# pdeljanov/Symphonia

Measured on AMD Instinct MI355X. Metric: decoded audio frames/sec (batch IMDCT+OLA), higher is better.
Workload: dtype f32

## Files before the change

### symphonia_amd/csrc/aac.hip

```cpp
#include <type_traits>

#include "imdct_wave.h"

namespace symaccel {

namespace {

#ifndef SYM_AAC_VARIANT
#define SYM_AAC_VARIANT 0
#endif
#if SYM_AAC_VARIANT == 1
constexpr int kWaves = 6;
#define SYM_AAC_WAVES_PER_SIMD 3
#else
constexpr int kWaves = 4;
#endif
constexpr int kTabTw = 0;
constexpr int kTabKbd = 1024;
constexpr int kTabSine = 2048;
constexpr int kTabKbdShort = 3072;
constexpr int kTabSineShort = 3200;
constexpr int kTabFloats = 3328;

enum : int { ONLY_LONG = 0, LONG_START = 1, EIGHT_SHORT = 2, LONG_STOP = 3 };
constexpr int kP0 = 512 - 64;
constexpr int kP1 = 512 + 64;

__device__ __forceinline__ void pcm_short4(const float *H, int q0, const float *short_win, const float *prev_short_win,
                                           float (&acc)[4]) {
    const int w = q0 >> 7, i0 = q0 & 127;
    bool have = false;
    if (w >= 1) {
        float a[4];
        ys4(H, w - 1, 128 + i0, a);
        const float4 wr = *reinterpret_cast<const float4 *>(short_win + 124 - i0);
        a[0] *= wr.w; a[1] *= wr.z; a[2] *= wr.y; a[3] *= wr.x;
#pragma unroll
        for (int q = 0; q < 4; ++q) acc[q] = (w - 1 == 0) ? a[q] : (0.0f + a[q]);
        have = true;
    }
    if (w <= 7) {
        float bq[4];
        ys4(H, w, i0, bq);
        const float4 wf = *reinterpret_cast<const float4 *>((w == 0 ? prev_short_win : short_win) + i0);
        bq[0] *= wf.x; bq[1] *= wf.y; bq[2] *= wf.z; bq[3] *= wf.w;
#pragma unroll
        for (int q = 0; q < 4; ++q) acc[q] = have ? (acc[q] + bq[q]) : bq[q];
    }
}

__device__ __forceinline__ void stop_window4(const float *psw, int j0, float *w) {
    float4 v = make_float4(1.0f, 1.0f, 1.0f, 1.0f);
    if (j0 >= kP0 && j0 < kP1) v = *reinterpret_cast<const float4 *>(psw + j0 - kP0);
    w[0] = v.x; w[1] = v.y; w[2] = v.z; w[3] = v.w;
}
__device__ __forceinline__ void start_window4(const float *sw, int j0, float *w) {
    float4 v = make_float4(1.0f, 1.0f, 1.0f, 1.0f);
    if (j0 >= kP0 && j0 < kP1) {
        const float4 r = *reinterpret_cast<const float4 *>(sw + 124 - (j0 - kP0));
        v = make_float4(r.w, r.z, r.y, r.x);
    }
    w[0] = v.x; w[1] = v.y; w[2] = v.z; w[3] = v.w;
}

#if defined(SYM_AAC_WAVES_PER_SIMD) && !defined(SYM_AAC_MIN_WAVES)
#define SYM_AAC_MIN_WAVES SYM_AAC_WAVES_PER_SIMD
#endif
#ifndef SYM_AAC_MIN_WAVES
#define SYM_AAC_MIN_WAVES 2
#endif
#ifndef SYM_AAC_PREFETCH
#define SYM_AAC_PREFETCH 1
#endif
#ifndef SYM_AAC_QUAD
#define SYM_AAC_QUAD 1
#endif
__device__ __forceinline__ float2 ld_line(const float2 *p) { return ld_stream(p); }
__device__ __forceinline__ void st_slot(float *frame, int m2, const float (&v)[8]) {
    float4 *o4 = reinterpret_cast<float4 *>(frame);
    st_stream(o4 + m2, make_float4(v[0], v[1], v[2], v[3]));
    st_stream(o4 + 255 - m2, make_float4(v[4], v[5], v[6], v[7]));
}


#if !SYM_AAC_QUAD
#include "experiments/aac_wave_walk.h"
#endif



constexpr int kSlotOff = kShortRowsEnd;
static_assert(kSlotOff + 1024 <= kWaveLds, "delay slot must fit the per-wave LDS behind the short-window rows");

struct AacJsArgs {
    const int2 *chain;
    const int32_t *pair_chains;
    const symaccel_aac_js_frame *desc;
    AacBandMaps maps;
    unsigned n_chains;
};

template <bool JS>
__global__ __launch_bounds__(256, SYM_AAC_MIN_WAVES) void aac_synth_quad_kernel(
    DevTables tb, const float *__restrict__ coeffs, const uint8_t *__restrict__ side,
    const float *__restrict__ delay_in, float *__restrict__ delay_out, float *__restrict__ pcm,
    unsigned frames_per_chain, unsigned seg_steps, unsigned segs_per_chain, AacJsArgs js) {
    __shared__ __attribute__((aligned(16))) float tabs[kTabFloats];
    __shared__ __attribute__((aligned(16))) float wave_lds[4][kWaveLds];
    constexpr int CH = JS ? 2 : 1;
    __shared__ __attribute__((aligned(16))) float carry[CH][2][1024];
    if constexpr (!JS) {
        if (js.chain && js.chain[blockIdx.x / segs_per_chain].x >= 0) return;
    }
    for (int i = (int)threadIdx.x; i < 1024; i += 256) {
        tabs[kTabTw + i] = reinterpret_cast<const float *>(tb.aac_tw_long)[i];
        tabs[kTabKbd + i] = tb.aac_kbd_long[i];
        tabs[kTabSine + i] = tb.aac_sine_long[i];
        if (i < 128) {
            tabs[kTabKbdShort + i] = tb.aac_kbd_short[i];
            tabs[kTabSineShort + i] = tb.aac_sine_short[i];
        }
    }
    const int lane = (int)threadIdx.x & 63, wave = (int)threadIdx.x >> 6;
    float *ldsf = wave_lds[wave];
    c32 *lds = reinterpret_cast<c32 *>(ldsf);
    const c32 *tw = reinterpret_cast<const c32 *>(tabs + kTabTw);
    const unsigned unit = blockIdx.x / segs_per_chain, seg = blockIdx.x % segs_per_chain;
    const unsigned chain = JS ? (unsigned)js.pair_chains[2 * unit] : unit, chain1 = JS ? (unsigned)js.pair_chains[2 * unit + 1] : unit;
    if constexpr (JS) {
        if (chain >= js.n_chains || chain1 >= js.n_chains || chain == chain1) return;
    }
    const long t_begin = (long)seg * seg_steps * 4;
    const long t_end = t_begin + (long)seg_steps * 4 < (long)frames_per_chain ? t_begin + (long)seg_steps * 4 : (long)frames_per_chain;
    const long n_steps = (t_end - t_begin + 3) / 4;
    const size_t chain_base0 = (size_t)chain * frames_per_chain, chain_base1 = (size_t)chain1 * frames_per_chain;
    LaneTables lt;
    load_lane_tables(tb, lane, lt);

    if (t_begin == 0 && wave == 3) {
#pragma unroll
        for (int ch = 0; ch < CH; ++ch) {
            const float4 *src = reinterpret_cast<const float4 *>(delay_in + (size_t)(ch ? chain1 : chain) * 1024);
#pragma unroll
            for (int q = 0; q < 4; ++q) reinterpret_cast<float4 *>(carry[ch][1])[lane + 64 * q] = src[lane + 64 * q];
        }
    }
    long t_loaded = (wave == 3 && t_begin > 0) ? t_begin - 1 : t_begin + wave;
    float2 line[8];
    unsigned sb_next = 0;
    float2 line1[8];
    uint32_t dq[3] = {0u, 0u, 0u};
    unsigned sb1_next = 0;
    uint32_t sfb_long[2] = {0u, 0u};
    unsigned sfb_short = 0;
    auto fetch1 = [&](long tf, int ln) {
        if constexpr (JS) {
            const float2 *ps = reinterpret_cast<const float2 *>(coeffs + (chain_base1 + (size_t)tf) * 1024);
            const uint32_t *d = reinterpret_cast<const uint32_t *>(js.desc + (size_t)unit * frames_per_chain + (size_t)tf);
#pragma unroll
            for (int s = 0; s < 8; ++s) line1[s] = ld_line(ps + ln + 64 * s);
            dq[0] = d[ln];
            dq[1] = d[ln + 64];
            dq[2] = ln < 33 ? d[ln + 128] : 0u;
            sb1_next = side[chain_base1 + (size_t)tf];
        }
    };
    if constexpr (JS) {
#pragma unroll
        for (int s = 0; s < 8; ++s) sfb_long[s >> 2] |= (uint32_t)js.maps.long4[(lane >> 1) + 32 * s] << (8 * (s & 3));
        sfb_short = js.maps.short4[(lane >> 1) & 31];
    }
    if (t_loaded < t_end) {
        const float2 *src = reinterpret_cast<const float2 *>(coeffs + (chain_base0 + (size_t)t_loaded) * 1024);
#pragma unroll
        for (int s = 0; s < 8; ++s) line[s] = ld_line(src + lane + 64 * s);
        sb_next = side[chain_base0 + (size_t)t_loaded];
        fetch1(t_loaded, lane);
    } else {
        t_loaded = -100;
#pragma unroll
        for (int s = 0; s < 8; ++s) line[s] = make_float2(0.0f, 0.0f);
        if constexpr (JS) {
#pragma unroll
            for (int s = 0; s < 8; ++s) line1[s] = make_float2(0.0f, 0.0f);
        }
    }
    __syncthreads();

    long t = t_begin - 4 + wave;
    const int lane_of_wave = lane;
    for (long i = -1; i < n_steps; ++i, t += 4) {
        int lane = lane_of_wave;
        if constexpr (JS) {
#if defined(__HIP_DEVICE_COMPILE__)
            asm volatile("" : "+v"(lane));
#endif
        }
        const bool active = t == t_loaded;
        const bool emit = i >= 0;
        const unsigned sb0 = sb_next, sb1 = sb1_next;
        if constexpr (JS) {
            if (active) {
                uint32_t *dl = reinterpret_cast<uint32_t *>(ldsf);
                dl[lane] = dq[0];
                dl[lane + 64] = dq[1];
                if (lane < 33) dl[lane + 128] = dq[2];
                wave_sync();
                const unsigned hdr = dl[0];
                const bool one = (hdr & 255u) == 1u;
                const int max_sfb = (int)((hdr >> 8) & 255u);
                const uint8_t *mode = reinterpret_cast<const uint8_t *>(dl + 1);
                const float *scale = reinterpret_cast<const float *>(dl + 33);
#pragma unroll
                for (int s = 0; s < 8; ++s) {
                    const float2 l = line[s], r = line1[s];
                    const int sfb = one ? (int)((sfb_long[s >> 2] >> (8 * (s & 3))) & 255u) : (int)sfb_short;
                    const int slot = one ? sfb : 16 * s + sfb;
                    const bool coded = sfb < max_sfb && slot < 128;
                    const int sl = slot < 127 ? slot : 127;
                    const unsigned m = mode[sl];
                    const float sc = scale[sl];
                    const bool ms = coded && m == SYMACCEL_AAC_JS_MS, is = coded && m == SYMACCEL_AAC_JS_INTENSITY;
                    line[s] = ms ? make_float2(l.x + r.x, l.y + r.y) : l;
                    line1[s] = ms ? make_float2(l.x - r.x, l.y - r.y) : (is ? make_float2(sc * l.x, sc * l.y) : r);
                }
                wave_sync();
            }
        }
        const long tn = t < t_begin ? t_begin + 3 : t + 4;
#pragma unroll 1
        for (int ch = 0; ch < CH; ++ch) {
        if constexpr (JS) {
#if defined(__HIP_DEVICE_COMPILE__)
            asm volatile("" : "+v"(lane));
#endif
        }
        const unsigned sb = ch ? sb1 : sb0;
        const size_t chain_base = ch ? chain_base1 : chain_base0;
        const int seq = (int)(sb & 3u);
        const int shape = (int)((sb >> 2) & 1u), prev_shape = (int)((sb >> 3) & 1u);
        float *my_slot = wave == 3 ? carry[ch][i & 1] : ldsf + kSlotOff;
        const float *prev_slot = wave == 0 ? carry[ch][(i + 1) & 1] : wave_lds[wave - 1] + kSlotOff;
        float xw[2][8];
        auto ln_at = [&](int s) -> float2 {
            if constexpr (JS) return ch ? line1[s] : line[s];
            else return line[s];
        };

        if (active) {
            c32 z[8];
            if (seq != EIGHT_SHORT) {
                const int mirror = (63 - lane) * 4;
#pragma unroll
                for (int s = 0; s < 8; ++s) {
                    const float mirrored = __int_as_float(__builtin_amdgcn_ds_bpermute(mirror, __float_as_int(ln_at(7 - s).y)));
                    z[s] = pre_twiddle(ln_at(s).x, mirrored, tw[lane + 64 * s]);
                }
            } else {
#pragma unroll
                for (int s = 0; s < 8; ++s) {
                    ldsf[short_row(s) + 2 * lane] = ln_at(s).x;
                    ldsf[short_row(s) + 2 * lane + 1] = ln_at(s).y;
                }
                wave_sync();
            }
            if (tn < t_end) {
                if (ch == 0) {
                    sb_next = side[chain_base0 + (size_t)tn];
                    const float2 *src = reinterpret_cast<const float2 *>(coeffs + (chain_base0 + (size_t)tn) * 1024);
#pragma unroll
                    for (int s = 0; s < 8; ++s) line[s] = ld_line(src + lane + 64 * s);
                }
                if (ch == CH - 1) fetch1(tn, lane);
            }
            if (seq != EIGHT_SHORT) {
                fft512_wave(z, lane, lds, lt);
                const float *wprev = tabs + (prev_shape ? kTabKbd : kTabSine);
                const float *wcur = tabs + (shape ? kTabKbd : kTabSine);
#pragma unroll
                for (int h = 0; h < 2; ++h) {
                    const int m2 = lane + 64 * h;
                    float x[8], x2[8];
                    post_slot(lds, tw, m2, x, x2);
                    float wo[8];
                    if (seq == LONG_STOP) {
                        const float *psw = tabs + (prev_shape ? kTabKbdShort : kTabSineShort);
                        stop_window4(psw, 4 * m2, wo);
                        stop_window4(psw, 1020 - 4 * m2, wo + 4);
                    } else {
                        load_slot(wprev, m2, wo);
                    }
#pragma unroll
                    for (int q = 0; q < 8; ++q) xw[h][q] = x[q] * wo[q];
                    float wd[8], nd[8];
                    if (seq == LONG_START) {
                        const float *sw = tabs + (shape ? kTabKbdShort : kTabSineShort);
                        start_window4(sw, 4 * m2, wd);
                        start_window4(sw, 1020 - 4 * m2, wd + 4);
                    } else {
                        float wr[8];
                        load_slot(wcur, m2, wr);
#pragma unroll
                        for (int q = 0; q < 8; ++q) wd[q] = wr[7 - q];
                    }
#pragma unroll
                    for (int q = 0; q < 8; ++q) {
                        const int j = q < 4 ? 4 * m2 + q : 1020 - 4 * m2 + (q - 4);
                        const float v = x2[q] * wd[q];
                        nd[q] = (seq == LONG_START && j >= kP1) ? 0.0f : v;
                    }
                    store_slot(my_slot, m2, nd);
                }
            } else {
                imdct_short_wave(lane, ldsf, tb.aac_tw_short, lt);
                const float *sw = tabs + (shape ? kTabKbdShort : kTabSineShort);
                const float *psw = tabs + (prev_shape ? kTabKbdShort : kTabSineShort);
#pragma unroll 1
                for (int e = 0; e < 4; ++e) {
                    const int j0 = 4 * lane + 256 * e;
                    float nd[4] = {0.0f, 0.0f, 0.0f, 0.0f};
                    if (j0 < kP1) pcm_short4(ldsf, j0 + kP1, sw, psw, nd);
                    *reinterpret_cast<float4 *>(my_slot + j0) = make_float4(nd[0], nd[1], nd[2], nd[3]);
                }
            }
        }
        wg_sync_lds();

        if (active && emit) {
            float *frame_out = pcm + (chain_base + (size_t)t) * 1024;
            if (seq != EIGHT_SHORT) {
#pragma unroll
                for (int h = 0; h < 2; ++h) {
                    const int m2 = lane + 64 * h;
                    float dl[8], dst[8];
                    load_slot(prev_slot, m2, dl);
#pragma unroll
                    for (int q = 0; q < 8; ++q) {
                        const int j = q < 4 ? 4 * m2 + q : 1020 - 4 * m2 + (q - 4);
                        const float v = dl[q] + xw[h][q];
                        dst[q] = (seq == LONG_STOP && j < kP0) ? dl[q] : v;
                    }
                    st_slot(frame_out, m2, dst);
                }
            } else {
                const float *sw = tabs + (shape ? kTabKbdShort : kTabSineShort);
                const float *psw = tabs + (prev_shape ? kTabKbdShort : kTabSineShort);
#pragma unroll 1
                for (int e = 0; e < 4; ++e) {
                    const int j0 = 4 * lane + 256 * e;
                    const float4 d = *reinterpret_cast<const float4 *>(prev_slot + j0);
                    float o[4] = {d.x, d.y, d.z, d.w};
                    if (j0 >= kP0) {
                        float ps[4];
                        pcm_short4(ldsf, j0 - kP0, sw, psw, ps);
#pragma unroll
                        for (int q = 0; q < 4; ++q) o[q] = o[q] + ps[q];
                    }
                    st_stream(reinterpret_cast<float4 *>(frame_out + j0), make_float4(o[0], o[1], o[2], o[3]));
                }
            }
            if (t + 1 == (long)frames_per_chain) {
                float4 *d = reinterpret_cast<float4 *>(delay_out + (size_t)(ch ? chain1 : chain) * 1024);
#pragma unroll
                for (int q = 0; q < 4; ++q) d[lane + 64 * q] = reinterpret_cast<const float4 *>(my_slot)[lane + 64 * q];
            }
        }
        wg_sync_lds();
        }
        if (active) t_loaded = tn < t_end ? tn : -100;
    }
}

__global__ void aac_js_index_kernel(const int32_t *__restrict__ pair_chains, unsigned n_pairs, unsigned n_chains, int2 *__restrict__ chain_index) {
    const unsigned i = blockIdx.x * blockDim.x + threadIdx.x;
    if (i < 2 * n_pairs && (unsigned)pair_chains[i] < n_chains && (unsigned)pair_chains[i ^ 1u] < n_chains)
        chain_index[pair_chains[i]] = make_int2(pair_chains[i ^ 1u], (int)i);
}

}

int launch_aac(symaccel_ctx *ctx, const float *d_coeffs, const uint8_t *d_side, const float *d_delay_in,
               float *d_delay_out, float *d_pcm, size_t n_chains, size_t frames_per_chain, const AacBandMaps *maps,
               const int32_t *d_pair_chains, const symaccel_aac_js_frame *d_js_desc, size_t n_pairs, void *d_js_scratch) {
    if (frames_per_chain > 0x7fffffffu) return SYMACCEL_ERR_INVALID_ARG;
#if SYM_AAC_QUAD
    {
        const size_t steps_per_chain = (frames_per_chain + 3) / 4;
        unsigned seg_steps;
        if (ctx->segment > 0) seg_steps = (unsigned)((ctx->segment + 3) / 4);
        else seg_steps = choose_segment(ctx, n_chains, steps_per_chain, SYM_AAC_MIN_WAVES, 1, 1, 1);
        if (seg_steps > steps_per_chain) seg_steps = (unsigned)steps_per_chain;
        const size_t segs = (steps_per_chain + seg_steps - 1) / seg_steps;
        const size_t grid = n_chains * segs;
        if (grid > 0x7fffffffu) return SYMACCEL_ERR_INVALID_ARG;
        AacJsArgs js{nullptr, nullptr, nullptr, AacBandMaps{}, (unsigned)n_chains};
        if (n_pairs == 0 || !maps) {
            hipLaunchKernelGGL(aac_synth_quad_kernel<false>, dim3((unsigned)grid), dim3(256), 0, ctx->stream, ctx->dev, d_coeffs, d_side,
                               d_delay_in, d_delay_out, d_pcm, (unsigned)frames_per_chain, seg_steps, (unsigned)segs, js);
        } else {
            if (n_pairs * frames_per_chain > 0x7fffffffu) return SYMACCEL_ERR_INVALID_ARG;
            const bool unpaired = 2 * n_pairs < n_chains;
            int2 *chain_index = unpaired ? reinterpret_cast<int2 *>(d_js_scratch) : nullptr;
            if (unpaired) {
                SYM_GPU(ctx, hipMemsetAsync(chain_index, 0xff, n_chains * sizeof(int2), ctx->stream));
                hipLaunchKernelGGL(aac_js_index_kernel, dim3((unsigned)((2 * n_pairs + 255) / 256)), dim3(256), 0, ctx->stream, d_pair_chains,
                                   (unsigned)n_pairs, (unsigned)n_chains, chain_index);
                SYM_GPU(ctx, hipGetLastError());
            }
            js = AacJsArgs{chain_index, d_pair_chains, d_js_desc, *maps, (unsigned)n_chains};
            unsigned pseg_steps;
            if (ctx->segment > 0) pseg_steps = (unsigned)((ctx->segment + 3) / 4);
            else pseg_steps = choose_segment(ctx, n_pairs, steps_per_chain, SYM_AAC_MIN_WAVES, 1, 1, 1);
            if (pseg_steps > steps_per_chain) pseg_steps = (unsigned)steps_per_chain;
            const size_t psegs = (steps_per_chain + pseg_steps - 1) / pseg_steps;
            if (n_pairs * psegs > 0x7fffffffu) return SYMACCEL_ERR_INVALID_ARG;
            hipLaunchKernelGGL(aac_synth_quad_kernel<true>, dim3((unsigned)(n_pairs * psegs)), dim3(256), 0, ctx->stream, ctx->dev, d_coeffs, d_side,
                               d_delay_in, d_delay_out, d_pcm, (unsigned)frames_per_chain, pseg_steps, (unsigned)psegs, js);
            SYM_GPU(ctx, hipGetLastError());
            if (unpaired)
                hipLaunchKernelGGL(aac_synth_quad_kernel<false>, dim3((unsigned)grid), dim3(256), 0, ctx->stream, ctx->dev, d_coeffs, d_side,
                                   d_delay_in, d_delay_out, d_pcm, (unsigned)frames_per_chain, seg_steps, (unsigned)segs, js);
        }
        SYM_GPU(ctx, hipGetLastError());
        return SYMACCEL_OK;
    }
#else
    return launch_aac_wave_walk(ctx, d_coeffs, d_side, d_delay_in, d_delay_out, d_pcm, n_chains, frames_per_chain);
#endif
}

}
```

Baseline: 305.4 million.

## Split quad synth loop into halo, full and ragged steps with specialized tails

Restructures the per-wave step loop into a templated step lambda called as a halo step, a loop of full steps, and a ragged tail. The per-step active, emit and bound checks disappear, and the halo step needs only a wave sync instead of a workgroup barrier. The long-window tail is specialized per window sequence, reusing the previous window when the shapes match. The short-window output is staged through LDS so all paths share one store. It adds readfirstlane scalarization, a scheduling barrier that forces the prefetch to settle, and an optional probe header, at the cost of code size and register pressure.

```diff
diff --git a/symphonia_amd/csrc/aac.hip b/symphonia_amd/csrc/aac.hip
--- a/symphonia_amd/csrc/aac.hip
+++ b/symphonia_amd/csrc/aac.hip
@@ -92,6 +92,17 @@
 constexpr int kSlotOff = kShortRowsEnd;
 static_assert(kSlotOff + 1024 <= kWaveLds, "delay slot must fit the per-wave LDS behind the short-window rows");
 
+enum : int { kStepHalo = 0, kStepFull = 1, kStepRagged = 2 };
+template <int V> using step_kind = std::integral_constant<int, V>;
+
+__device__ __forceinline__ void settle_prefetch(const float2 (&line)[8]) {
+#if defined(__HIP_DEVICE_COMPILE__)
+    __builtin_amdgcn_sched_barrier(0);
+    asm volatile("" : : "v"(line[0].x), "v"(line[0].y), "v"(line[1].x), "v"(line[1].y), "v"(line[2].x), "v"(line[2].y), "v"(line[3].x), "v"(line[3].y),
+                        "v"(line[4].x), "v"(line[4].y), "v"(line[5].x), "v"(line[5].y), "v"(line[6].x), "v"(line[6].y), "v"(line[7].x), "v"(line[7].y));
+#endif
+}
+
 struct AacJsArgs {
     const int2 *chain;
     const int32_t *pair_chains;
@@ -99,6 +110,10 @@
     AacBandMaps maps;
     unsigned n_chains;
 };
+
+#if SYM_AAC_QUAD == 2
+#include "experiments/aac_quad_probe.h"
+#endif
 
 template <bool JS>
 __global__ __launch_bounds__(256, SYM_AAC_MIN_WAVES) void aac_synth_quad_kernel(
@@ -121,7 +136,7 @@
             tabs[kTabSineShort + i] = tb.aac_sine_short[i];
         }
     }
-    const int lane = (int)threadIdx.x & 63, wave = (int)threadIdx.x >> 6;
+    const int lane = (int)threadIdx.x & 63, wave = __builtin_amdgcn_readfirstlane((int)threadIdx.x >> 6);
     float *ldsf = wave_lds[wave];
     c32 *lds = reinterpret_cast<c32 *>(ldsf);
     const c32 *tw = reinterpret_cast<const c32 *>(tabs + kTabTw);
@@ -132,12 +147,13 @@
     }
     const long t_begin = (long)seg * seg_steps * 4;
     const long t_end = t_begin + (long)seg_steps * 4 < (long)frames_per_chain ? t_begin + (long)seg_steps * 4 : (long)frames_per_chain;
-    const long n_steps = (t_end - t_begin + 3) / 4;
+    if (t_end <= t_begin) return;
     const size_t chain_base0 = (size_t)chain * frames_per_chain, chain_base1 = (size_t)chain1 * frames_per_chain;
     LaneTables lt;
     load_lane_tables(tb, lane, lt);
 
-    if (t_begin == 0 && wave == 3) {
+    const bool has_halo = t_begin > 0;
+    if (!has_halo && wave == 3) {
 #pragma unroll
         for (int ch = 0; ch < CH; ++ch) {
             const float4 *src = reinterpret_cast<const float4 *>(delay_in + (size_t)(ch ? chain1 : chain) * 1024);
@@ -145,7 +161,7 @@
             for (int q = 0; q < 4; ++q) reinterpret_cast<float4 *>(carry[ch][1])[lane + 64 * q] = src[lane + 64 * q];
         }
     }
-    long t_loaded = (wave == 3 && t_begin > 0) ? t_begin - 1 : t_begin + wave;
+    const long t_first = (wave == 3 && has_halo) ? t_begin - 1 : t_begin + wave;
     float2 line[8];
     unsigned sb_next = 0;
     float2 line1[8];
@@ -170,14 +186,13 @@
         for (int s = 0; s < 8; ++s) sfb_long[s >> 2] |= (uint32_t)js.maps.long4[(lane >> 1) + 32 * s] << (8 * (s & 3));
         sfb_short = js.maps.short4[(lane >> 1) & 31];
     }
-    if (t_loaded < t_end) {
-        const float2 *src = reinterpret_cast<const float2 *>(coeffs + (chain_base0 + (size_t)t_loaded) * 1024);
+    if (t_first < t_end) {
+        const float2 *src = reinterpret_cast<const float2 *>(coeffs + (chain_base0 + (size_t)t_first) * 1024);
 #pragma unroll
         for (int s = 0; s < 8; ++s) line[s] = ld_line(src + lane + 64 * s);
-        sb_next = side[chain_base0 + (size_t)t_loaded];
-        fetch1(t_loaded, lane);
+        sb_next = side[chain_base0 + (size_t)t_first];
+        fetch1(t_first, lane);
     } else {
-        t_loaded = -100;
 #pragma unroll
         for (int s = 0; s < 8; ++s) line[s] = make_float2(0.0f, 0.0f);
         if constexpr (JS) {
@@ -187,18 +202,17 @@
     }
     __syncthreads();
 
-    long t = t_begin - 4 + wave;
     const int lane_of_wave = lane;
-    for (long i = -1; i < n_steps; ++i, t += 4) {
+    auto step = [&](auto kind_c, int i, long t, bool active) __attribute__((always_inline)) {
+        constexpr int KIND = decltype(kind_c)::value;
         int lane = lane_of_wave;
         if constexpr (JS) {
 #if defined(__HIP_DEVICE_COMPILE__)
             asm volatile("" : "+v"(lane));
 #endif
         }
-        const bool active = t == t_loaded;
-        const bool emit = i >= 0;
-        const unsigned sb0 = sb_next, sb1 = sb1_next;
+        const unsigned sb0 = (unsigned)__builtin_amdgcn_readfirstlane((int)sb_next);
+        const unsigned sb1 = JS ? (unsigned)__builtin_amdgcn_readfirstlane((int)sb1_next) : 0u;
         if constexpr (JS) {
             if (active) {
                 uint32_t *dl = reinterpret_cast<uint32_t *>(ldsf);
@@ -227,7 +241,8 @@
                 wave_sync();
             }
         }
-        const long tn = t < t_begin ? t_begin + 3 : t + 4;
+        const long tn = KIND == kStepHalo ? t_begin + 3 : (t + 4 < t_end ? t + 4 : t);
+        const bool fetch = KIND == kStepFull || (KIND == kStepHalo && tn < t_end);
 #pragma unroll 1
         for (int ch = 0; ch < CH; ++ch) {
         if constexpr (JS) {
@@ -240,12 +255,56 @@
         const int seq = (int)(sb & 3u);
         const int shape = (int)((sb >> 2) & 1u), prev_shape = (int)((sb >> 3) & 1u);
         float *my_slot = wave == 3 ? carry[ch][i & 1] : ldsf + kSlotOff;
-        const float *prev_slot = wave == 0 ? carry[ch][(i + 1) & 1] : wave_lds[wave - 1] + kSlotOff;
+        float *prev_slot = wave == 0 ? carry[ch][(i + 1) & 1] : wave_lds[wave > 0 ? wave - 1 : 0] + kSlotOff;
         float xw[2][8];
         auto ln_at = [&](int s) -> float2 {
             if constexpr (JS) return ch ? line1[s] : line[s];
             else return line[s];
         };
+        auto long_tail = [&](auto seq_c) __attribute__((always_inline)) {
+            constexpr int SEQ = decltype(seq_c)::value;
+            const float *wprev = tabs + (prev_shape ? kTabKbd : kTabSine);
+            const float *wcur = tabs + (shape ? kTabKbd : kTabSine);
+#pragma unroll
+            for (int h = 0; h < 2; ++h) {
+                const int m2 = lane + 64 * h;
+                float x[8], x2[8];
+                post_slot(lds, tw, m2, x, x2);
+                float wo[8];
+                if constexpr (SEQ == LONG_STOP) {
+                    const float *psw = tabs + (prev_shape ? kTabKbdShort : kTabSineShort);
+                    stop_window4(psw, 4 * m2, wo);
+                    stop_window4(psw, 1020 - 4 * m2, wo + 4);
+                } else {
+                    load_slot(wprev, m2, wo);
+                }
+#pragma unroll
+                for (int q = 0; q < 8; ++q) xw[h][q] = x[q] * wo[q];
+                float wd[8], nd[8];
+                if constexpr (SEQ == LONG_START) {
+                    const float *sw = tabs + (shape ? kTabKbdShort : kTabSineShort);
+                    start_window4(sw, 4 * m2, wd);
+                    start_window4(sw, 1020 - 4 * m2, wd + 4);
+                } else {
+                    float wr[8];
+                    if (SEQ == ONLY_LONG && shape == prev_shape) {
+#pragma unroll
+                        for (int q = 0; q < 8; ++q) wr[q] = wo[q];
+                    } else {
+                        load_slot(wcur, m2, wr);
+                    }
+#pragma unroll
+                    for (int q = 0; q < 8; ++q) wd[q] = wr[7 - q];
+                }
+#pragma unroll
+                for (int q = 0; q < 8; ++q) {
+                    const int j = q < 4 ? 4 * m2 + q : 1020 - 4 * m2 + (q - 4);
+                    const float v = x2[q] * wd[q];
+                    nd[q] = (SEQ == LONG_START && j >= kP1) ? 0.0f : v;
+                }
+                store_slot(my_slot, m2, nd);
+            }
+        };
 
         if (active) {
             c32 z[8];
@@ -264,7 +323,7 @@
                 }
                 wave_sync();
             }
-            if (tn < t_end) {
+            if (fetch) {
                 if (ch == 0) {
                     sb_next = side[chain_base0 + (size_t)tn];
                     const float2 *src = reinterpret_cast<const float2 *>(coeffs + (chain_base0 + (size_t)tn) * 1024);
@@ -275,42 +334,9 @@
             }
             if (seq != EIGHT_SHORT) {
                 fft512_wave(z, lane, lds, lt);
-                const float *wprev = tabs + (prev_shape ? kTabKbd : kTabSine);
-                const float *wcur = tabs + (shape ? kTabKbd : kTabSine);
-#pragma unroll
-                for (int h = 0; h < 2; ++h) {
-                    const int m2 = lane + 64 * h;
-                    float x[8], x2[8];
-                    post_slot(lds, tw, m2, x, x2);
-                    float wo[8];
-                    if (seq == LONG_STOP) {
-                        const float *psw = tabs + (prev_shape ? kTabKbdShort : kTabSineShort);
-                        stop_window4(psw, 4 * m2, wo);
-                        stop_window4(psw, 1020 - 4 * m2, wo + 4);
-                    } else {
-                        load_slot(wprev, m2, wo);
-                    }
-#pragma unroll
-                    for (int q = 0; q < 8; ++q) xw[h][q] = x[q] * wo[q];
-                    float wd[8], nd[8];
-                    if (seq == LONG_START) {
-                        const float *sw = tabs + (shape ? kTabKbdShort : kTabSineShort);
-                        start_window4(sw, 4 * m2, wd);
-                        start_window4(sw, 1020 - 4 * m2, wd + 4);
-                    } else {
-                        float wr[8];
-                        load_slot(wcur, m2, wr);
-#pragma unroll
-                        for (int q = 0; q < 8; ++q) wd[q] = wr[7 - q];
-                    }
-#pragma unroll
-                    for (int q = 0; q < 8; ++q) {
-                        const int j = q < 4 ? 4 * m2 + q : 1020 - 4 * m2 + (q - 4);
-                        const float v = x2[q] * wd[q];
-                        nd[q] = (seq == LONG_START && j >= kP1) ? 0.0f : v;
-                    }
-                    store_slot(my_slot, m2, nd);
-                }
+                if (seq == ONLY_LONG) long_tail(step_kind<ONLY_LONG>{});
+                else if (seq == LONG_START) long_tail(step_kind<LONG_START>{});
+                else long_tail(step_kind<LONG_STOP>{});
             } else {
                 imdct_short_wave(lane, ldsf, tb.aac_tw_short, lt);
                 const float *sw = tabs + (shape ? kTabKbdShort : kTabSineShort);
@@ -324,23 +350,29 @@
                 }
             }
         }
+        if constexpr (KIND == kStepHalo) {
+            wave_sync();
+        } else {
         wg_sync_lds();
 
-        if (active && emit) {
+        if (active) {
             float *frame_out = pcm + (chain_base + (size_t)t) * 1024;
+            float dst[2][8];
             if (seq != EIGHT_SHORT) {
 #pragma unroll
                 for (int h = 0; h < 2; ++h) {
                     const int m2 = lane + 64 * h;
-                    float dl[8], dst[8];
+                    float dl[8];
                     load_slot(prev_slot, m2, dl);
 #pragma unroll
-                    for (int q = 0; q < 8; ++q) {
-                        const int j = q < 4 ? 4 * m2 + q : 1020 - 4 * m2 + (q - 4);
-                        const float v = dl[q] + xw[h][q];
-                        dst[q] = (seq == LONG_STOP && j < kP0) ? dl[q] : v;
+                    for (int q = 0; q < 8; ++q) dst[h][q] = dl[q] + xw[h][q];
+                    if (seq == LONG_STOP) {
+#pragma unroll
+                        for (int q = 0; q < 8; ++q) {
+                            const int j = q < 4 ? 4 * m2 + q : 1020 - 4 * m2 + (q - 4);
+                            dst[h][q] = j < kP0 ? dl[q] : dst[h][q];
+                        }
                     }
-                    st_slot(frame_out, m2, dst);
                 }
             } else {
                 const float *sw = tabs + (shape ? kTabKbdShort : kTabSineShort);
@@ -356,9 +388,15 @@
 #pragma unroll
                         for (int q = 0; q < 4; ++q) o[q] = o[q] + ps[q];
                     }
-                    st_stream(reinterpret_cast<float4 *>(frame_out + j0), make_float4(o[0], o[1], o[2], o[3]));
-                }
-            }
+                    *reinterpret_cast<float4 *>(prev_slot + j0) = make_float4(o[0], o[1], o[2], o[3]);
+                }
+                wave_sync();
+#pragma unroll
+                for (int h = 0; h < 2; ++h) load_slot(prev_slot, lane + 64 * h, dst[h]);
+            }
+#pragma unroll
+            for (int h = 0; h < 2; ++h) st_slot(frame_out, lane + 64 * h, dst[h]);
+            if constexpr (KIND == kStepFull && !JS) settle_prefetch(line);
             if (t + 1 == (long)frames_per_chain) {
                 float4 *d = reinterpret_cast<float4 *>(delay_out + (size_t)(ch ? chain1 : chain) * 1024);
 #pragma unroll
@@ -367,8 +405,16 @@
         }
         wg_sync_lds();
         }
-        if (active) t_loaded = tn < t_end ? tn : -100;
-    }
+        }
+    };
+
+    if (has_halo && wave == 3) step(step_kind<kStepHalo>{}, -1, t_begin - 1, true);
+    if constexpr (!JS) settle_prefetch(line);
+    const int n_full = (int)((t_end - t_begin) >> 2);
+    long t = t_begin + wave;
+#pragma unroll 1
+    for (int i = 0; i < n_full; ++i, t += 4) step(step_kind<kStepFull>{}, i, t, true);
+    if ((t_end - t_begin) & 3) step(step_kind<kStepRagged>{}, n_full, t, t < t_end);
 }
 
 __global__ void aac_js_index_kernel(const int32_t *__restrict__ pair_chains, unsigned n_pairs, unsigned n_chains, int2 *__restrict__ chain_index) {
diff --git a/symphonia_amd/csrc/experiments/aac_quad_probe.h b/symphonia_amd/csrc/experiments/aac_quad_probe.h
--- /dev/null
+++ b/symphonia_amd/csrc/experiments/aac_quad_probe.h
@@ -0,0 +1,62 @@
+#pragma once
+
+struct QuadProbeAcc {
+    unsigned long long pairs, b1, b2, wait, t0, calls, pad0, pad1;
+};
+
+__device__ __forceinline__ QuadProbeAcc *quad_probe_acc(int wave) {
+    __shared__ QuadProbeAcc acc[4];
+    return &acc[wave & 3];
+}
+
+__device__ __forceinline__ void quad_probe_begin(int wave, int lane) {
+    QuadProbeAcc *a = quad_probe_acc(wave);
+    if (lane == 0) {
+        a->pairs = a->b1 = a->b2 = a->wait = a->calls = 0ull;
+        a->t0 = __builtin_readcyclecounter();
+    }
+    (__syncthreads)();
+}
+
+__device__ __forceinline__ void quad_probe_sync(int wave, int lane, float *first_frame) {
+    QuadProbeAcc *a = quad_probe_acc(wave);
+    const unsigned long long c0 = __builtin_readcyclecounter();
+    (wg_sync_lds)();
+    const unsigned long long c1 = __builtin_readcyclecounter();
+    if (lane == 0) {
+        const unsigned long long k = a->calls;
+        a->calls = k + 1;
+        if ((k & 1ull) == 0ull) {
+            a->b1 += c1 - c0;
+        } else {
+            a->b2 += c1 - c0;
+            const unsigned long long pairs = a->pairs + 1;
+            a->pairs = pairs;
+            if ((pairs & 31ull) == 0ull) {
+                unsigned hw, xcc;
+                asm volatile("s_getreg_b32 %0, hwreg(HW_REG_HW_ID)" : "=s"(hw));
+                asm volatile("s_getreg_b32 %0, hwreg(HW_REG_XCC_ID)" : "=s"(xcc));
+                uint4 *o = reinterpret_cast<uint4 *>(first_frame) + 4 * (wave & 3);
+                o[0] = make_uint4(0x57e9c10cu, (unsigned)pairs, (unsigned)a->b1, (unsigned)a->b2);
+                o[1] = make_uint4((unsigned)a->wait, (unsigned)(c1 - a->t0), hw, xcc);
+            }
+        }
+    }
+}
+
+template <typename Claim>
+__device__ __forceinline__ void quad_probe_wait(int wave, int lane, Claim claim) {
+    const unsigned long long c0 = __builtin_readcyclecounter();
+    claim();
+    const unsigned long long c1 = __builtin_readcyclecounter();
+    if (lane == 0) quad_probe_acc(wave)->wait += c1 - c0;
+}
+
+#define __syncthreads() quad_probe_begin(wave, lane)
+#define wg_sync_lds() quad_probe_sync(wave, lane, pcm + (chain_base0 + (size_t)t_begin) * 1024)
+#define settle_prefetch(l) quad_probe_wait(wave, lane, [&]() { (settle_prefetch)(l); })
+#define SYM_PROBE_TOP(l, sb)                                                                                                     \
+    quad_probe_wait(wave, lane, [&]() {                                                                                          \
+        asm volatile("" : : "v"(l[0].x), "v"(l[0].y), "v"(l[1].x), "v"(l[1].y), "v"(l[2].x), "v"(l[2].y), "v"(l[3].x), "v"(l[3].y), \
+                     "v"(l[4].x), "v"(l[4].y), "v"(l[5].x), "v"(l[5].y), "v"(l[6].x), "v"(l[6].y), "v"(l[7].x), "v"(l[7].y), "v"(sb)); \
+    })
```

Measured after the change: 329.3 million, median of 6. 7.8% higher.
